# ZechengLi19/CIM

Measured on AMD Instinct MI355X. Metric: images/sec training step (ResNet-50 VOC, ~1k proposals/img) at 1/2/4/8 GPU, higher is better.
Workload: dtype fp32

## Files before the change

cim_amd/csrc/conv1x1.hip:

```cpp
#include "common.h"
#include "../../include/cim_hip.h"

#ifndef CIM_BODY_PRIO_LEVEL
#define CIM_BODY_PRIO_LEVEL 3
#endif
#if CIM_BODY_PRIO_LEVEL > 0
#define CIM_BODY_PRIO() __builtin_amdgcn_s_setprio(CIM_BODY_PRIO_LEVEL)
#else
#define CIM_BODY_PRIO()
#endif
namespace {

#ifndef CIM_SMALL_BK
#define CIM_SMALL_BK 32
#endif
#ifndef CIM_SMALL_ABL
#define CIM_SMALL_ABL 0
#endif
constexpr int SBM = 64, SBN = 64, SBK = CIM_SMALL_BK;
constexpr int SLD = 68;
typedef float f32x16 __attribute__((ext_vector_type(16)));
typedef float f32x4u __attribute__((ext_vector_type(4), aligned(4)));
__device__ __forceinline__ float4 ld4(const float* p) {
    const f32x4u v = *reinterpret_cast<const f32x4u*>(p);
    return make_float4(v.x, v.y, v.z, v.w);
}

struct SmallArgs {
    const float* A; const float* B; float* C; float* Xraw;
    const float* gamma; const float* beta; const float* mean; const float* var; const float* res;
    float eps;
    int M, N, K, lda, ldb, ldc;
    int a_mcontig, b_kcontig, relu, bn;
    int splits; float* ws;
    const float* colbias;
    const float* mask; const float* mgamma; const float* mvar; float meps;
    const float* mxr; const float* mmean; float* mpart; int mparts;
    int res_w, res_ws, res_hw;
};
struct InputBn { const float* y; const float* gamma; const float* var; float eps;
                 const float* xr; const float* mean; float* part; };

typedef unsigned int u32x4 __attribute__((ext_vector_type(4)));
typedef __amdgpu_buffer_rsrc_t rsrc_t;
__device__ __forceinline__ rsrc_t make_rsrc(const float* p, long long floats) {
    return __builtin_amdgcn_make_buffer_rsrc(const_cast<float*>(p), 0, (int)(unsigned)(floats * 4), 0x00020000);
}
__device__ __forceinline__ float4 bld4(rsrc_t r, unsigned byte_off) {
    const u32x4 v = __builtin_amdgcn_raw_buffer_load_b128(r, byte_off, 0, 0);
    return make_float4(__uint_as_float(v.x), __uint_as_float(v.y), __uint_as_float(v.z), __uint_as_float(v.w));
}
__device__ __forceinline__ float bld1(rsrc_t r, unsigned byte_off) {
    return __uint_as_float(__builtin_amdgcn_raw_buffer_load_b32(r, byte_off, 0, 0));
}
constexpr unsigned OOB = 0x7fffffffu;
__host__ __device__ __forceinline__ long long tile_extent(bool RC, int rows, int K, int ld) {
    return RC ? (long long)(K - 1) * ld + rows : (long long)(rows - 1) * ld + K;
}
template <bool RC, int ROWS>
__device__ __forceinline__ unsigned tile_off(int ld, int r0, int k0, int p) {
    int r, k;
    if (RC) { k = k0 + p / (ROWS / 4); r = r0 + (p % (ROWS / 4)) * 4; return ((unsigned)k * ld + r) * 4u; }
    r = r0 + p % ROWS; k = k0 + (p / ROWS) * 4;
    return ((unsigned)r * ld + k) * 4u;
}
template <bool RC, int ROWS>
__device__ __forceinline__ float4 tile_ktail(float4 v, int K, int k0, int p) {
    if (!RC) {
        const int left = K - (k0 + (p / ROWS) * 4);
        v.x = left > 0 ? v.x : 0.0f; v.y = left > 1 ? v.y : 0.0f; v.z = left > 2 ? v.z : 0.0f; v.w = left > 3 ? v.w : 0.0f;
    }
    return v;
}

template <bool RC, int ROWS>
__device__ __forceinline__ void tile_store(float* __restrict__ S, float4 v, int p) {
    if (RC) {
        const int k = p / (ROWS / 4), r = (p % (ROWS / 4)) * 4;
        *reinterpret_cast<float4*>(S + k * SLD + r) = v;
    } else {
        const int r = p % ROWS, k = (p / ROWS) * 4;
        S[(k + 0) * SLD + r] = v.x;
        S[(k + 1) * SLD + r] = v.y;
        S[(k + 2) * SLD + r] = v.z;
        S[(k + 3) * SLD + r] = v.w;
    }
}

__device__ __forceinline__ float small_value(const SmallArgs& g, int row, int col, float v, float& s1, float& s2) {
    const size_t o = (size_t)row * g.ldc + col;
    float y = v;
    if (g.bn) {
        const float a = g.gamma[row] * rsqrtf(g.var[row] + g.eps);
        y = fmaf(v, a, g.beta[row] - g.mean[row] * a);
    }
    if (g.res) {
        if (g.res_w == 0) y += g.res[o];
        else {
            const int py = col / g.res_w, px = col - py * g.res_w;
            if (!((py | px) & 1)) y += g.res[(size_t)row * g.res_hw + (py >> 1) * g.res_ws + (px >> 1)];
        }
    }
    if (g.colbias) y += g.colbias[col];
    if (g.relu) y = fmaxf(y, 0.0f);
    if (g.mask) {
        const bool on = g.mask[o] > 0.0f;
        if (g.mpart && on) { s1 += y; s2 = fmaf(y, g.mxr[o] - g.mmean[row], s2); }
        y = on ? y * (g.mgamma[row] * rsqrtf(g.mvar[row] + g.meps)) : 0.0f;
    }
    return y;
}
__device__ __forceinline__ void small_finish(const SmallArgs& g, int row, int col, float v, float& s1, float& s2) {
    const size_t o = (size_t)row * g.ldc + col;
    if (g.Xraw) g.Xraw[o] = v;
    g.C[o] = small_value(g, row, col, v, s1, s2);
}
__device__ __forceinline__ void small_finish(const SmallArgs& g, int row, int col, float v) {
    float s1 = 0.0f, s2 = 0.0f;
    small_finish(g, row, col, v, s1, s2);
}
__device__ __forceinline__ void small_put_part(const SmallArgs& g, int row, int group, int lane, float s1, float s2) {
#pragma unroll
    for (int o = 16; o > 0; o >>= 1) {
        s1 += __shfl_xor(s1, o);
        s2 += __shfl_xor(s2, o);
    }
    if ((lane & 31) == 0 && row < g.M && group < g.mparts) {
        g.mpart[(size_t)group * g.M + row] = s1;
        g.mpart[((size_t)g.mparts + group) * g.M + row] = s2;
    }
}
__device__ __forceinline__ void small_epilogue(const SmallArgs& g, const f32x16& acc, int row0, int col0, int lane, int split) {
    const int col = col0 + (lane & 31);
    if (g.splits > 1) {
        if (col < g.N) {
#pragma unroll
            for (int r = 0; r < 16; ++r) {
                const int row = row0 + 8 * (r >> 2) + 4 * (lane >> 5) + (r & 3);
                if (row < g.M) g.ws[((size_t)split * g.M + row) * g.N + col] = acc[r];
            }
        }
        return;
    }
    if (g.mpart == nullptr) {
        if (col < g.N) {
#pragma unroll
            for (int r = 0; r < 16; ++r) {
                const int row = row0 + 8 * (r >> 2) + 4 * (lane >> 5) + (r & 3);
                if (row < g.M) small_finish(g, row, col, acc[r]);
            }
        }
        return;
    }
#pragma unroll
    for (int r = 0; r < 16; ++r) {
        const int row = row0 + 8 * (r >> 2) + 4 * (lane >> 5) + (r & 3);
        float s1 = 0.0f, s2 = 0.0f;
        if (col < g.N && row < g.M) small_finish(g, row, col, acc[r], s1, s2);
        small_put_part(g, row, col0 >> 5, lane, s1, s2);
    }
}


template <bool AM, bool BKc, int WN>
__global__ __launch_bounds__(128 * WN) void gemm_small_kernel(const SmallArgs g) {
    CIM_BODY_PRIO();
    constexpr int NT = 128 * WN, BNT = 32 * WN;
    constexpr int PA = SBM * 8 / NT, PB = BNT * 8 / NT;
    __shared__ __attribute__((aligned(16))) float As[2][SBK * SLD];
    __shared__ __attribute__((aligned(16))) float Bs[2][SBK * SLD];
    const int tid = threadIdx.x, lane = tid & 63, wave = tid >> 6;
    const int wm = wave / WN, wn = wave % WN;
    const int tiles_n = (g.N + BNT - 1) / BNT;
    const int tile = blockIdx.x;
    const int m0 = (tile / tiles_n) * SBM, n0 = (tile % tiles_n) * BNT;
    const int split = blockIdx.y;
    const int kper = ((g.K + g.splits - 1) / g.splits + SBK - 1) / SBK * SBK;
    const int kbeg = split * kper, kend = min(g.K, kbeg + kper);
#if CIM_SMALL_ABL == 4
    if (g.M > 0) return;
#endif

    f32x16 acc;
#pragma unroll
    for (int i = 0; i < 16; ++i) acc[i] = 0.0f;

    const rsrc_t RA_ = make_rsrc(g.A, tile_extent(AM, g.M, g.K, g.lda)), RB_ = make_rsrc(g.B, tile_extent(!BKc, g.N, g.K, g.ldb));
    unsigned oa[PA], ob[PB];
#pragma unroll
    for (int i = 0; i < PA; ++i) oa[i] = tile_off<AM, SBM>(g.lda, m0, kbeg, tid + i * NT);
#pragma unroll
    for (int i = 0; i < PB; ++i) ob[i] = tile_off<!BKc, BNT>(g.ldb, n0, kbeg, tid + i * NT);
    const unsigned sa = (AM ? (unsigned)g.lda * SBK : (unsigned)SBK) * 4u, sb = (!BKc ? (unsigned)g.ldb * SBK : (unsigned)SBK) * 4u;
    float4 ra0[PA], rb0[PB], ra1[PA], rb1[PB];
#if CIM_SMALL_ABL == 3
#define SM_GLOAD(RA, RB, S)                                                                                        \
    {                                                                                                              \
        _Pragma("unroll") for (int i = 0; i < PA; ++i) asm volatile("" : "+v"(RA[i].x), "+v"(RA[i].y), "+v"(RA[i].z), "+v"(RA[i].w)); \
        _Pragma("unroll") for (int i = 0; i < PB; ++i) asm volatile("" : "+v"(RB[i].x), "+v"(RB[i].y), "+v"(RB[i].z), "+v"(RB[i].w)); \
    }
#else
#define SM_GLOAD(RA, RB, S)                                                                                        \
    {                                                                                                              \
        _Pragma("unroll") for (int i = 0; i < PA; ++i) RA[i] = bld4(RA_, oa[i] + (unsigned)(S) * sa);               \
        _Pragma("unroll") for (int i = 0; i < PB; ++i) RB[i] = bld4(RB_, ob[i] + (unsigned)(S) * sb);               \
    }
#endif
#define SM_PUT(RA, RB, BUF, S)                                                                                     \
    {                                                                                                              \
        _Pragma("unroll") for (int i = 0; i < PA; ++i)                                                             \
            tile_store<AM, SBM>(As[BUF], tile_ktail<AM, SBM>(RA[i], g.K, kbeg + (S) * SBK, tid + i * NT), tid + i * NT);     \
        _Pragma("unroll") for (int i = 0; i < PB; ++i)                                                             \
            tile_store<!BKc, BNT>(Bs[BUF], tile_ktail<!BKc, BNT>(RB[i], g.K, kbeg + (S) * SBK, tid + i * NT), tid + i * NT); \
    }
#define SM_MMA(BUF)                                                                                                \
    {                                                                                                              \
        const float* __restrict__ a = As[BUF] + (lane >> 5) * SLD + wm * 32 + (lane & 31);                         \
        const float* __restrict__ b = Bs[BUF] + (lane >> 5) * SLD + wn * 32 + (lane & 31);                         \
        float av[SBK / 2], bv[SBK / 2];                                                                            \
        _Pragma("unroll") for (int t = 0; t < SBK / 2; ++t) { av[t] = a[2 * t * SLD]; bv[t] = b[2 * t * SLD]; }    \
        _Pragma("unroll") for (int t = 0; t < (CIM_SMALL_ABL == 1 ? 1 : SBK / 2); ++t)                             \
            acc = __builtin_amdgcn_mfma_f32_32x32x2f32(av[t], bv[t], acc, 0, 0, 0);                                \
        asm volatile("" : "+a"(acc));       \
    }
    if (kbeg < kend) {
        const int nslab = (kend - kbeg + SBK - 1) / SBK;
        const int last = nslab - 1;
        SM_GLOAD(ra0, rb0, 0)
        SM_GLOAD(ra1, rb1, min(1, last))
        SM_PUT(ra0, rb0, 0, 0)
        asm volatile("" : "+a"(acc));
        __syncthreads();
        for (int s = 0; s < nslab; s += 2) {
            SM_GLOAD(ra0, rb0, min(s + 2, last))
            SM_MMA(0)
            if (s + 1 < nslab) SM_PUT(ra1, rb1, 1, s + 1)
            __syncthreads();
            if (s + 1 >= nslab) break;
            SM_GLOAD(ra1, rb1, min(s + 3, last))
            SM_MMA(1)
            if (s + 2 < nslab) SM_PUT(ra0, rb0, 0, s + 2)
            __syncthreads();
        }
    }
#undef SM_GLOAD
#undef SM_PUT
#undef SM_MMA

#if CIM_SMALL_ABL == 2
    if (m0 + wm * 32 + lane < 0) small_epilogue(g, acc, m0 + wm * 32, n0 + wn * 32, lane, split);
#else
    small_epilogue(g, acc, m0 + wm * 32, n0 + wn * 32, lane, split);
#endif
}

__device__ __forceinline__ float splitk_sum(const float* __restrict__ ws, size_t i, size_t mn, int splits) {
    float v = ws[i];
    for (int k0 = 1; k0 < splits; k0 += 8) {
        float p[8];
#pragma unroll
        for (int j = 0; j < 8; ++j) p[j] = k0 + j < splits ? ws[(size_t)(k0 + j) * mn + i] : 0.0f;
#pragma unroll
        for (int j = 0; j < 8; ++j)
            if (k0 + j < splits) v += p[j];
    }
    return v;
}
__global__ __launch_bounds__(256) void small_splitk_reduce_kernel(const SmallArgs g) {
    CIM_BODY_PRIO();
    const size_t i = (size_t)blockIdx.x * 256 + threadIdx.x;
    const size_t mn = (size_t)g.M * g.N;
    if (i >= mn) return;
    small_finish(g, (int)(i / g.N), (int)(i % g.N), splitk_sum(g.ws, i, mn, g.splits));
}
__global__ __launch_bounds__(256) void small_splitk_reduce4_kernel(const SmallArgs g) {
    CIM_BODY_PRIO();
    const size_t q = (size_t)blockIdx.x * 256 + threadIdx.x;
    const size_t mn = (size_t)g.M * g.N;
    const size_t i = q * 4;
    if (i >= mn) return;
    float4 v = *reinterpret_cast<const float4*>(g.ws + i);
    for (int k0 = 1; k0 < g.splits; k0 += 4) {
        float4 p[4];
#pragma unroll
        for (int j = 0; j < 4; ++j)
            p[j] = k0 + j < g.splits ? *reinterpret_cast<const float4*>(g.ws + (size_t)(k0 + j) * mn + i) : make_float4(0.f, 0.f, 0.f, 0.f);
#pragma unroll
        for (int j = 0; j < 4; ++j)
            if (k0 + j < g.splits) { v.x += p[j].x; v.y += p[j].y; v.z += p[j].z; v.w += p[j].w; }
    }
    int row = (int)(i / g.N), col = (int)(i - (size_t)row * g.N);
    const float s[4] = {v.x, v.y, v.z, v.w};
    float y[4], s1 = 0.0f, s2 = 0.0f;
#pragma unroll
    for (int j = 0; j < 4; ++j) {
        y[j] = small_value(g, row, col, s[j], s1, s2);
        if (++col == g.N) { col = 0; ++row; }
    }
    if (g.Xraw) *reinterpret_cast<float4*>(g.Xraw + i) = v;
    *reinterpret_cast<float4*>(g.C + i) = make_float4(y[0], y[1], y[2], y[3]);
}

__global__ __launch_bounds__(256) void small_splitk_reduce_rows_kernel(const SmallArgs g) {
    CIM_BODY_PRIO();
    const int col = blockIdx.x * 256 + threadIdx.x, row = blockIdx.y;
    const size_t mn = (size_t)g.M * g.N;
    float s1 = 0.0f, s2 = 0.0f;
    if (col < g.N) {
        const size_t i = (size_t)row * g.N + col;
        small_finish(g, row, col, splitk_sum(g.ws, i, mn, g.splits), s1, s2);
    }
    small_put_part(g, row, col >> 5, threadIdx.x & 63, s1, s2);
}

struct BnPartTable { cim_bn_part_desc d[24]; int first[25]; int n; };
__global__ __launch_bounds__(256) void bn_part_finish_kernel(const BnPartTable t) {
    CIM_BODY_PRIO();
    __shared__ float sh[2][8][32];
    int e = 0;
    while (e + 1 < t.n && (int)blockIdx.x >= t.first[e + 1]) ++e;
    const cim_bn_part_desc& d = t.d[e];
    const int C = d.channels, parts = d.parts, total = d.images * d.parts;
    const int c = ((int)blockIdx.x - t.first[e]) * 32 + (threadIdx.x & 31), grp = threadIdx.x >> 5;
    float t1 = 0.0f, t2 = 0.0f;
    if (c < C) {
        for (int i0 = grp; i0 < total; i0 += 32) {
            float a[4], b[4];
#pragma unroll
            for (int j = 0; j < 4; ++j) {
                const int i = i0 + 8 * j;
                const int img = i / parts, p = i - img * parts;
                const float* q = d.part + ((size_t)img * 2 * parts + p) * C + c;
                a[j] = i < total ? q[0] : 0.0f;
                b[j] = i < total ? q[(size_t)parts * C] : 0.0f;
            }
#pragma unroll
            for (int j = 0; j < 4; ++j) { t1 += a[j]; t2 += b[j]; }
        }
    }
    sh[0][grp][threadIdx.x & 31] = t1;
    sh[1][grp][threadIdx.x & 31] = t2;
    __syncthreads();
    if (grp == 0 && c < C) {
        float a1 = 0.0f, a2 = 0.0f;
#pragma unroll
        for (int k = 0; k < 8; ++k) { a1 += sh[0][k][threadIdx.x]; a2 += sh[1][k][threadIdx.x]; }
        if (d.dbeta) d.dbeta[c] = a1;
        if (d.dgamma) d.dgamma[c] = a2 * rsqrtf(d.var[c] + d.eps);
    }
}

enum { CONV_FWD = 0, CONV_DX = 1, CONV_DW = 2 };
struct ConvGeom { int H, W, Ho, Wo, stride, cin, cout; float inv_w; int dil; };

#ifndef CIM_CONV3_BK
#define CIM_CONV3_BK 32
#endif
constexpr int CBK = CIM_CONV3_BK;
template <int MODE, int KS = 3>
__global__ __launch_bounds__(256) void conv3x3_small_kernel(const SmallArgs g, const ConvGeom c) {
    CIM_BODY_PRIO();
    constexpr int TAPS = KS * KS;
    constexpr int NT = 256, PA = SBM * (CBK / 4) / NT, PB = SBN * (CBK / 4) / NT;
    extern __shared__ __attribute__((aligned(16))) float c3_smem[];
    float (*As)[CBK * SLD] = reinterpret_cast<float (*)[CBK * SLD]>(c3_smem);
    float (*Bs)[CBK * SLD] = reinterpret_cast<float (*)[CBK * SLD]>(c3_smem + 2 * CBK * SLD);
    const int tid = threadIdx.x, lane = tid & 63, wave = tid >> 6;
    const int wm = wave >> 1, wn = wave & 1;
    const int tiles_n = (g.N + SBN - 1) / SBN;
    const int m0 = (blockIdx.x / tiles_n) * SBM, n0 = (blockIdx.x % tiles_n) * SBN;
    const int split = blockIdx.y;
    const int kper = ((g.K + g.splits - 1) / g.splits + CBK - 1) / CBK * CBK;
    const int kbeg = split * kper, kend = min(g.K, kbeg + kper);

    const rsrc_t RA_ = make_rsrc(g.A, tile_extent(MODE == CONV_DX, g.M, g.K, g.lda));
    const rsrc_t RB_ = make_rsrc(g.B, (long long)(MODE == CONV_DX ? c.cout * c.Ho * c.Wo : c.cin * c.H * c.W));
    const int hw_src = MODE == CONV_DX ? c.Ho * c.Wo : c.H * c.W;
    int py[PB][4], px[PB][4];
    int boff[PB], bdy[PB], bdx[PB];
#pragma unroll
    for (int i = 0; i < PB; ++i) {
        const int p = tid + i * NT;
        if (MODE == CONV_DW) {
            const int n = n0 + p % SBN;
            const int ch = n / TAPS, tap = n - ch * TAPS;
            boff[i] = n < g.N ? ch * hw_src : -1;
            bdy[i] = (tap / KS - KS / 2) * c.dil;
            bdx[i] = (tap - (tap / KS) * KS - KS / 2) * c.dil;
        } else {
            const int wrow = (MODE == CONV_DX) ? c.W : c.Wo;
#pragma unroll
            for (int j = 0; j < 4; ++j) {
                const int n = n0 + (p % 16) * 4 + j;
                const int y = (int)(((float)n + 0.5f) * c.inv_w);
                py[i][j] = n < g.N ? y : -(1 << 20);
                px[i][j] = n - y * wrow;
            }
        }
    }
    unsigned oa[PA];
#pragma unroll
    for (int i = 0; i < PA; ++i) oa[i] = tile_off<MODE == CONV_DX, SBM>(g.lda, m0, kbeg, tid + i * NT);
    const unsigned sa = (MODE == CONV_DX ? (unsigned)g.lda * CBK : (unsigned)CBK) * 4u;

    auto load_b = [&](int k0, float4 (&rb)[PB]) {
#pragma unroll
        for (int i = 0; i < PB; ++i) {
            const int p = tid + i * NT;
            unsigned off[4];
            if (MODE == CONV_DW) {
                const int k = k0 + (p / SBN) * 4;
#pragma unroll
                for (int j = 0; j < 4; ++j) {
                    const int po = k + j;
                    const int yo = (int)(((float)po + 0.5f) * c.inv_w), xo = po - yo * c.Wo;
                    const int yi = yo * c.stride + bdy[i], xi = xo * c.stride + bdx[i];
                    const bool ok = boff[i] >= 0 && po < g.K && (unsigned)yi < (unsigned)c.H && (unsigned)xi < (unsigned)c.W;
                    off[j] = ok ? (unsigned)(boff[i] + yi * c.W + xi) * 4u : OOB;
                }
            } else {
                const int k = k0 + p / 16;
                const int ch = k / TAPS, tap = k - ch * TAPS;
                const int dy = (tap / KS - KS / 2) * c.dil, dx = (tap - (tap / KS) * KS - KS / 2) * c.dil;
                const int base = ch * hw_src;
#pragma unroll
                for (int j = 0; j < 4; ++j) {
                    if (MODE == CONV_DX) {
                        const int ty = py[i][j] - dy, tx = px[i][j] - dx;
                        const int yo = c.stride == 2 ? ty >> 1 : ty, xo = c.stride == 2 ? tx >> 1 : tx;
                        const bool ok = ty >= 0 && tx >= 0 && yo < c.Ho && xo < c.Wo && !(c.stride == 2 && ((ty | tx) & 1));
                        off[j] = ok ? (unsigned)(base + yo * c.Wo + xo) * 4u : OOB;
                    } else {
                        const int yi = py[i][j] * c.stride + dy, xi = px[i][j] * c.stride + dx;
                        const bool ok = (unsigned)yi < (unsigned)c.H && (unsigned)xi < (unsigned)c.W;
                        off[j] = ok ? (unsigned)(base + yi * c.W + xi) * 4u : OOB;
                    }
                }
            }
#if CIM_SMALL_ABL == 3
            asm volatile("" : "+v"(rb[i].x), "+v"(rb[i].y), "+v"(rb[i].z), "+v"(rb[i].w) : "v"(off[0]), "v"(off[1]), "v"(off[2]), "v"(off[3]));
#elif CIM_SMALL_ABL == 5
            rb[i] = make_float4(bld1(RB_, (unsigned)(p * 16 + k0 * 64)), bld1(RB_, (unsigned)(p * 16 + k0 * 64 + 4)),
                                bld1(RB_, (unsigned)(p * 16 + k0 * 64 + 8)), bld1(RB_, (unsigned)(p * 16 + k0 * 64 + 12)));
#else
            rb[i] = make_float4(bld1(RB_, off[0]), bld1(RB_, off[1]), bld1(RB_, off[2]), bld1(RB_, off[3]));
#endif
        }
    };
    auto load_a = [&](int s, float4 (&ra)[PA]) {
#pragma unroll
        for (int i = 0; i < PA; ++i)
            ra[i] = bld4(RA_, oa[i] + (unsigned)s * sa);
    };

    f32x16 acc;
#pragma unroll
    for (int i = 0; i < 16; ++i) acc[i] = 0.0f;
    float4 ra0[PA], rb0[PB], ra1[PA], rb1[PB];
#define C3_PUT(RA, RB, BUF, S)                                                                                      \
    {                                                                                                               \
        _Pragma("unroll") for (int i = 0; i < PA; ++i)                                                              \
            tile_store<MODE == CONV_DX, SBM>(As[BUF], tile_ktail<MODE == CONV_DX, SBM>(RA[i], g.K, kbeg + (S) * CBK, tid + i * NT), tid + i * NT); \
        _Pragma("unroll") for (int i = 0; i < PB; ++i) tile_store<MODE != CONV_DW, SBN>(Bs[BUF], RB[i], tid + i * NT); \
    }
#define C3_MMA(BUF)                                                                                                 \
    {                                                                                                               \
        const float* __restrict__ a = As[BUF] + (lane >> 5) * SLD + wm * 32 + (lane & 31);                          \
        const float* __restrict__ b = Bs[BUF] + (lane >> 5) * SLD + wn * 32 + (lane & 31);                          \
        float av[CBK / 2], bv[CBK / 2];                                                                             \
        _Pragma("unroll") for (int t = 0; t < CBK / 2; ++t) { av[t] = a[2 * t * SLD]; bv[t] = b[2 * t * SLD]; }     \
        _Pragma("unroll") for (int t = 0; t < (CIM_SMALL_ABL == 1 ? 1 : CBK / 2); ++t)                              \
            acc = __builtin_amdgcn_mfma_f32_32x32x2f32(av[t], bv[t], acc, 0, 0, 0);                                 \
        asm volatile("" : "+a"(acc));                                                                               \
    }
    if (kbeg < kend) {
        const int nslab = (kend - kbeg + CBK - 1) / CBK;
        const int last = nslab - 1;
        load_a(0, ra0); load_b(kbeg, rb0);
        load_a(min(1, last), ra1); load_b(kbeg + min(1, last) * CBK, rb1);
        C3_PUT(ra0, rb0, 0, 0)
        asm volatile("" : "+a"(acc));
        __syncthreads();
        for (int s = 0; s < nslab; s += 2) {
            load_a(min(s + 2, last), ra0); load_b(kbeg + min(s + 2, last) * CBK, rb0);
            C3_MMA(0)
            if (s + 1 < nslab) C3_PUT(ra1, rb1, 1, s + 1)
            __syncthreads();
            if (s + 1 >= nslab) break;
            load_a(min(s + 3, last), ra1); load_b(kbeg + min(s + 3, last) * CBK, rb1);
            C3_MMA(1)
            if (s + 2 < nslab) C3_PUT(ra0, rb0, 0, s + 2)
            __syncthreads();
        }
    }
#undef C3_PUT
#undef C3_MMA
#if CIM_SMALL_ABL == 2
    if (m0 + wm * 32 + lane < 0)
#endif
    small_epilogue(g, acc, m0 + wm * 32, n0 + wn * 32, lane, split);
}

struct Dx2Geom { int H, W, Ho, Wo, cin, cout; int first[5]; int tiles_n[4]; int group0[4]; };
struct ColMap { int Wc, W, py, px, Nc, group0; };

__device__ __forceinline__ void small_epilogue_mapped(const SmallArgs& g, const f32x16& acc, int row0, int col0, int lane, const ColMap& cm) {
    const int nc = col0 + (lane & 31);
    const bool in = nc < cm.Nc;
    const int yc = nc / cm.Wc, xc = nc - yc * cm.Wc;
    const int col = (2 * yc + cm.py) * cm.W + 2 * xc + cm.px;
    if (g.mpart == nullptr) {
        if (in) {
#pragma unroll
            for (int r = 0; r < 16; ++r) {
                const int row = row0 + 8 * (r >> 2) + 4 * (lane >> 5) + (r & 3);
                if (row < g.M) small_finish(g, row, col, acc[r]);
            }
        }
        return;
    }
#pragma unroll
    for (int r = 0; r < 16; ++r) {
        const int row = row0 + 8 * (r >> 2) + 4 * (lane >> 5) + (r & 3);
        float s1 = 0.0f, s2 = 0.0f;
        if (in && row < g.M) small_finish(g, row, col, acc[r], s1, s2);
        small_put_part(g, row, cm.group0 + (col0 >> 5), lane, s1, s2);
    }
}

__global__ __launch_bounds__(256) void conv3x3_dx2_kernel(const SmallArgs g, const Dx2Geom c) {
    CIM_BODY_PRIO();
    constexpr int NT = 256, PA = SBM * (CBK / 4) / NT, PB = SBN * (CBK / 4) / NT;
    extern __shared__ __attribute__((aligned(16))) float d2_smem[];
    float (*As)[CBK * SLD] = reinterpret_cast<float (*)[CBK * SLD]>(d2_smem);
    float (*Bs)[CBK * SLD] = reinterpret_cast<float (*)[CBK * SLD]>(d2_smem + 2 * CBK * SLD);
    const int tid = threadIdx.x, lane = tid & 63, wave = tid >> 6;
    const int wm = wave >> 1, wn = wave & 1;
    int cls = 0;
    while (cls < 3 && (int)blockIdx.x >= c.first[cls + 1]) ++cls;
    const int py = cls >> 1, px = cls & 1;
    const int Wc = (c.W - px + 1) >> 1, Nc = ((c.H - py + 1) >> 1) * Wc;
    const int local = (int)blockIdx.x - c.first[cls], tn = c.tiles_n[cls];
    const int m0 = (local / tn) * SBM, n0 = (local % tn) * SBN;
    const int nx = px ? 2 : 1, lgT = py + px, T = 1 << lgT;
    const int K = c.cout << lgT;
    const int nslab = (K + CBK - 1) / CBK;
    const int how = c.Ho * c.Wo;
    const rsrc_t RA_ = make_rsrc(g.A, tile_extent(true, g.M, 9 * c.cout, g.lda));
    const rsrc_t RB_ = make_rsrc(g.B, (long long)c.cout * how);
    int yc[PB][4], xc[PB][4];
#pragma unroll
    for (int i = 0; i < PB; ++i) {
        const int p = tid + i * NT;
#pragma unroll
        for (int j = 0; j < 4; ++j) {
            const int nc = n0 + (p % 16) * 4 + j;
            const int y = nc / Wc;
            yc[i][j] = nc < Nc ? y : -(1 << 20);
            xc[i][j] = nc - y * Wc;
        }
    }
    auto tap_of = [&](int j, int& tap, int& oy, int& ox) {
        const int jy = j / nx, jx = j - jy * nx;
        const int ky = py ? 2 * jy : 1, kx = px ? 2 * jx : 1;
        tap = ky * 3 + kx;
        oy = (py && jy == 0) ? 1 : 0;
        ox = (px && jx == 0) ? 1 : 0;
    };
    auto load_a = [&](int k0, float4 (&ra)[PA]) {
#pragma unroll
        for (int i = 0; i < PA; ++i) {
            const int p = tid + i * NT;
            const int k = k0 + p / (SBM / 4), r = m0 + (p % (SBM / 4)) * 4;
            const int co = k >> lgT;
            int tap, oy, ox;
            tap_of(k & (T - 1), tap, oy, ox);
            ra[i] = bld4(RA_, co < c.cout ? ((unsigned)(co * 9 + tap) * g.lda + r) * 4u : OOB);
        }
    };
    auto load_b = [&](int k0, float4 (&rb)[PB]) {
#pragma unroll
        for (int i = 0; i < PB; ++i) {
            const int p = tid + i * NT;
            const int k = k0 + p / 16;
            const int co = k >> lgT;
            int tap, oy, ox;
            tap_of(k & (T - 1), tap, oy, ox);
            const int base = co * how;
            unsigned off[4];
#pragma unroll
            for (int j = 0; j < 4; ++j) {
                const int yo = yc[i][j] + oy, xo = xc[i][j] + ox;
                const bool ok = co < c.cout && yo >= 0 && yo < c.Ho && xo < c.Wo;
                off[j] = ok ? (unsigned)(base + yo * c.Wo + xo) * 4u : OOB;
            }
            rb[i] = make_float4(bld1(RB_, off[0]), bld1(RB_, off[1]), bld1(RB_, off[2]), bld1(RB_, off[3]));
        }
    };
    f32x16 acc;
#pragma unroll
    for (int i = 0; i < 16; ++i) acc[i] = 0.0f;
    float4 ra0[PA], rb0[PB], ra1[PA], rb1[PB];
#define D2_PUT(RA, RB, BUF)                                                                                         \
    {                                                                                                               \
        _Pragma("unroll") for (int i = 0; i < PA; ++i) tile_store<true, SBM>(As[BUF], RA[i], tid + i * NT);          \
        _Pragma("unroll") for (int i = 0; i < PB; ++i) tile_store<true, SBN>(Bs[BUF], RB[i], tid + i * NT);          \
    }
#define D2_MMA(BUF)                                                                                                 \
    {                                                                                                               \
        const float* __restrict__ a = As[BUF] + (lane >> 5) * SLD + wm * 32 + (lane & 31);                          \
        const float* __restrict__ b = Bs[BUF] + (lane >> 5) * SLD + wn * 32 + (lane & 31);                          \
        float av[CBK / 2], bv[CBK / 2];                                                                             \
        _Pragma("unroll") for (int t = 0; t < CBK / 2; ++t) { av[t] = a[2 * t * SLD]; bv[t] = b[2 * t * SLD]; }     \
        _Pragma("unroll") for (int t = 0; t < CBK / 2; ++t)                                                         \
            acc = __builtin_amdgcn_mfma_f32_32x32x2f32(av[t], bv[t], acc, 0, 0, 0);                                 \
        asm volatile("" : "+a"(acc));                                                                               \
    }
    {
        const int last = nslab - 1;
        load_a(0, ra0); load_b(0, rb0);
        load_a(min(1, last) * CBK, ra1); load_b(min(1, last) * CBK, rb1);
        D2_PUT(ra0, rb0, 0)
        asm volatile("" : "+a"(acc));
        __syncthreads();
        for (int s = 0; s < nslab; s += 2) {
            load_a(min(s + 2, last) * CBK, ra0); load_b(min(s + 2, last) * CBK, rb0);
            D2_MMA(0)
            if (s + 1 < nslab) D2_PUT(ra1, rb1, 1)
            __syncthreads();
            if (s + 1 >= nslab) break;
            load_a(min(s + 3, last) * CBK, ra1); load_b(min(s + 3, last) * CBK, rb1);
            D2_MMA(1)
            if (s + 2 < nslab) D2_PUT(ra0, rb0, 0)
            __syncthreads();
        }
    }
#undef D2_PUT
#undef D2_MMA
    const ColMap cm{Wc, c.W, py, px, Nc, c.group0[cls]};
    small_epilogue_mapped(g, acc, m0 + wm * 32, n0 + wn * 32, lane, cm);
}

__global__ __launch_bounds__(256) void conv3x3_wt_kernel(const float* __restrict__ w, float* __restrict__ wt, int cin) {
    extern __shared__ float wt_s[];
    const int co = blockIdx.x, n = cin * 9;
    for (int i = threadIdx.x; i < n; i += 256) wt_s[i] = w[(size_t)co * n + i];
    __syncthreads();
    for (int i = threadIdx.x; i < n; i += 256) {
        const int tap = i / cin, ci = i - tap * cin;
        wt[(size_t)co * n + i] = wt_s[ci * 9 + tap];
    }
}

struct WtTable { cim_wt_desc d[16]; int first[17]; int n; };
__global__ __launch_bounds__(256) void conv3x3_wt_multi_kernel(const WtTable t) {
    extern __shared__ float wt_s[];
    int e = 0;
    while (e + 1 < t.n && (int)blockIdx.x >= t.first[e + 1]) ++e;
    const int co = blockIdx.x - t.first[e], cin = t.d[e].cin, n = cin * 9;
    const float* __restrict__ w = t.d[e].w;
    float* __restrict__ wt = t.d[e].wt;
    for (int i = threadIdx.x; i < n; i += 256) wt_s[i] = w[(size_t)co * n + i];
    __syncthreads();
    for (int i = threadIdx.x; i < n; i += 256) {
        const int tap = i / cin, ci = i - tap * cin;
        wt[(size_t)co * n + i] = wt_s[ci * 9 + tap];
    }
}

static void set_input_bn(SmallArgs& g, const InputBn* in_bn) {
    if (in_bn == nullptr) return;
    g.mask = in_bn->y; g.mgamma = in_bn->gamma; g.mvar = in_bn->var; g.meps = in_bn->eps;
    g.mxr = in_bn->xr; g.mmean = in_bn->mean; g.mpart = in_bn->part; g.mparts = (g.N + 31) / 32;
}
static void launch_splitk_reduce(const SmallArgs& g, hipStream_t st) {
    if (g.mpart) {
        hipLaunchKernelGGL(small_splitk_reduce_rows_kernel, dim3((unsigned)((g.N + 255) / 256), (unsigned)g.M), dim3(256), 0, st, g);
    } else {
        const size_t n = (size_t)g.M * g.N;
        if (n >= (1u << 19) && g.ldc == g.N && n % 4 == 0 && (((size_t)g.ws | (size_t)g.C | (size_t)g.Xraw) & 15) == 0)
            hipLaunchKernelGGL(small_splitk_reduce4_kernel, dim3((unsigned)((n / 4 + 255) / 256)), dim3(256), 0, st, g);
        else
            hipLaunchKernelGGL(small_splitk_reduce_kernel, dim3((unsigned)((n + 255) / 256)), dim3(256), 0, st, g);
    }
}

template <bool AM, bool BKc>
static void launch_small(const SmallArgs& g, int splits, hipStream_t st, bool narrow) {
    const long long tm = (g.M + SBM - 1) / SBM;
    if (narrow)
        hipLaunchKernelGGL((gemm_small_kernel<AM, BKc, 1>), dim3((unsigned)(tm * ((g.N + 31) / 32)), (unsigned)splits), dim3(128), 0, st, g);
    else
        hipLaunchKernelGGL((gemm_small_kernel<AM, BKc, 2>), dim3((unsigned)(tm * ((g.N + 63) / 64)), (unsigned)splits), dim3(256), 0, st, g);
}

}

extern "C" int cim_gemm_small_splits(int M, int N, int K) {
    const long long tiles = (long long)((M + SBM - 1) / SBM) * ((N + SBN - 1) / SBN);
#ifndef CIM_SMALL_WGS
#define CIM_SMALL_WGS 512
#endif
#ifndef CIM_SMALL_MINSLABS
#define CIM_SMALL_MINSLABS 4
#endif
    constexpr int min_k = CIM_SMALL_MINSLABS * SBK, want = CIM_SMALL_WGS;
    int s = 1;
    while (tiles * s < want && K / (s * 2) >= min_k && s < 64) s *= 2;
    return s;
}

static int gemm_small_impl(const float* A, const float* B, float* C, int M, int N, int K, int lda, int ldb, int ldc,
                           int a_mcontig, int b_kcontig, float* x_raw, const float* gamma, const float* beta,
                           const float* mean, const float* var, float eps, const float* residual, int relu, int splits,
                           float* workspace, void* stream, const InputBn* in_bn, int res_w = 0);

extern "C" int cim_gemm_small_f32(const float* A, const float* B, float* C, int M, int N, int K, int lda, int ldb, int ldc,
                                  int a_mcontig, int b_kcontig, float* x_raw, const float* gamma, const float* beta,
                                  const float* mean, const float* var, float eps, const float* residual, int relu, int splits,
                                  float* workspace, void* stream) {
    return gemm_small_impl(A, B, C, M, N, K, lda, ldb, ldc, a_mcontig, b_kcontig, x_raw, gamma, beta, mean, var, eps, residual, relu,
                           splits, workspace, stream, nullptr);
}

static int gemm_small_impl(const float* A, const float* B, float* C, int M, int N, int K, int lda, int ldb, int ldc,
                           int a_mcontig, int b_kcontig, float* x_raw, const float* gamma, const float* beta,
                           const float* mean, const float* var, float eps, const float* residual, int relu, int splits,
                           float* workspace, void* stream, const InputBn* in_bn, int res_w) {
    CIM_CHECK_ARG(res_w == 0 || (residual && res_w > 0 && N % res_w == 0 && ldc == N));
    CIM_CHECK_ARG(A && B && C && M > 0 && N > 0 && K > 0 && lda > 0 && ldb > 0 && ldc >= N && splits >= 1);
    CIM_CHECK_ARG((gamma == nullptr) == (beta == nullptr) && (gamma == nullptr) == (mean == nullptr) && (gamma == nullptr) == (var == nullptr));
    CIM_CHECK_ARG(splits == 1 || workspace);
    SmallArgs g{};
    g.A = A; g.B = B; g.C = C; g.Xraw = x_raw;
    g.gamma = gamma; g.beta = beta; g.mean = mean; g.var = var; g.res = residual; g.eps = eps;
    g.M = M; g.N = N; g.K = K; g.lda = lda; g.ldb = ldb; g.ldc = ldc;
    g.a_mcontig = a_mcontig; g.b_kcontig = b_kcontig; g.relu = relu; g.bn = gamma != nullptr;
    g.splits = splits; g.ws = workspace; g.colbias = nullptr;
    g.res_w = res_w;
    if (res_w) { g.res_ws = (res_w + 1) / 2; g.res_hw = ((N / res_w + 1) / 2) * g.res_ws; }
    set_input_bn(g, in_bn);
    const long long tiles = (long long)((M + SBM - 1) / SBM) * ((N + SBN - 1) / SBN);
    CIM_CHECK_ARG(tiles * 2 < (1ll << 31) && splits <= 65535 && M <= 65535);
    CIM_CHECK_ARG(tile_extent(a_mcontig != 0, M, K, lda) < (1ll << 29) && tile_extent(b_kcontig == 0, N, K, ldb) < (1ll << 29));
    const bool narrow = tiles * splits < 128;
    hipStream_t st = cim::as_stream(stream);
    if (a_mcontig) {
        if (b_kcontig) launch_small<true, true>(g, splits, st, narrow); else launch_small<true, false>(g, splits, st, narrow);
    } else {
        if (b_kcontig) launch_small<false, true>(g, splits, st, narrow); else launch_small<false, false>(g, splits, st, narrow);
    }
    if (splits > 1) launch_splitk_reduce(g, st);
    CIM_CHECK_LAUNCH();
    return 0;
}

extern "C" int cim_linear_bias_f32(const float* X, const float* W, const float* bias, float* Y, int M, int N, int K, int splits,
                                   float* workspace, void* stream) {
    CIM_CHECK_ARG(X && W && Y && M > 0 && N > 0 && K > 0 && splits >= 1 && splits <= 65535 && (splits == 1 || workspace));
    SmallArgs g{};
    g.A = X; g.B = W; g.C = Y; g.Xraw = nullptr;
    g.gamma = g.beta = g.mean = g.var = g.res = nullptr; g.eps = 0.f;
    g.M = M; g.N = N; g.K = K; g.lda = K; g.ldb = K; g.ldc = N;
    g.a_mcontig = 0; g.b_kcontig = 1; g.relu = 0; g.bn = 0;
    g.splits = splits; g.ws = workspace; g.colbias = bias;
    hipStream_t st = cim::as_stream(stream);
    launch_small<false, true>(g, splits, st, false);
    if (splits > 1) {
        const size_t n = (size_t)M * N;
        hipLaunchKernelGGL(small_splitk_reduce_kernel, dim3((unsigned)((n + 255) / 256)), dim3(256), 0, st, g);
    }
    CIM_CHECK_LAUNCH();
    return 0;
}

extern "C" long long cim_conv1x1_bwd_workspace(int B, int cin, int cout, int hw) {
    const long long dx = (long long)cim_gemm_small_splits(cin, hw, cout) * cin * hw;
    const long long dw = (long long)cim_gemm_small_splits(cout, cin, hw) * cout * cin + (B > 1 ? (long long)cout * cin : 0);
    const long long dconv = (long long)B * cout * hw;
    return (long long)sizeof(float) * (dconv + dx + dw);
}

namespace {
struct ForkJoin {
    hipStream_t main, side;
    hipEvent_t ev_fork, ev_join;
    bool on;
    ForkJoin(hipStream_t m, hipStream_t s, void* fork_event, void* join_event, bool want)
        : main(m), side(s), ev_fork(static_cast<hipEvent_t>(fork_event)), ev_join(static_cast<hipEvent_t>(join_event)),
          on(want && s != nullptr && s != m) {}
    hipStream_t fork() {
        if (!on) return main;
        (void)hipEventRecord(ev_fork, main);
        (void)hipStreamWaitEvent(side, ev_fork, 0);
        return side;
    }
    void join() {
        if (!on) return;
        (void)hipEventRecord(ev_join, side);
        (void)hipStreamWaitEvent(main, ev_join, 0);
    }
};

__global__ __launch_bounds__(256) void small_axpy_kernel(float* __restrict__ y, const float* __restrict__ x, size_t n) {
    const size_t i = (size_t)blockIdx.x * 256 + threadIdx.x;
    if (i < n) y[i] += x[i];
}
}

extern "C" int cim_conv1x1_bn_act_bwd(const float* dy, const float* y, const float* x_raw, const float* x, const float* w,
                                      const float* gamma, const float* mean, const float* var, float eps, int relu,
                                      float* dres, float* dgamma, float* dbeta, float* dx, float* dw, int B, int cin, int cout,
                                      int hw, float* workspace, void* stream, void* side_stream, void* fork_event, void* join_event, int join,
                                      int dy_is_dconv, const float* in_gamma, const float* in_var, float in_eps,
                                      const float* in_xr, const float* in_mean, float* in_part, const float* dx_add, int dx_add_w) {
    CIM_CHECK_ARG(dx_add_w == 0 || (dx_add != nullptr && dx_add_w > 0 && hw % dx_add_w == 0));
    CIM_CHECK_ARG(side_stream == nullptr || side_stream == stream || (fork_event != nullptr && (!join || join_event != nullptr)));
    const size_t add_bs = dx_add_w ? (size_t)cin * ((hw / dx_add_w + 1) / 2) * ((dx_add_w + 1) / 2) : (size_t)cin * hw;
    CIM_CHECK_ARG(dy && x_raw && x && w && gamma && mean && var && workspace && B > 0 && cin > 0 && cout > 0 && hw > 0);
    CIM_CHECK_ARG(dx_add == nullptr || (dx != nullptr && in_gamma == nullptr));
    CIM_CHECK_ARG((y != nullptr || !relu) && ((dgamma == nullptr) == (dbeta == nullptr)));
    CIM_CHECK_ARG(!dy_is_dconv || (dres == nullptr && dgamma == nullptr));
    CIM_CHECK_ARG((in_gamma == nullptr) == (in_var == nullptr));
    CIM_CHECK_ARG(in_part == nullptr || (in_gamma && in_xr && in_mean));
    float* dconv = dy_is_dconv ? const_cast<float*>(dy) : workspace;
    float* ws_dx = workspace + (size_t)B * cout * hw;
    float* ws_dw = ws_dx + (size_t)cim_gemm_small_splits(cin, hw, cout) * cin * hw;
    int rc = dy_is_dconv ? 0 : cim_bn_act_bwd(dy, y, x_raw, gamma, mean, var, eps, dconv, dres, dgamma, dbeta, B, cout, hw, relu, stream);
    if (rc) return rc;
    ForkJoin fj(cim::as_stream(stream), cim::as_stream(side_stream), fork_event, join_event, dx && dw);
    void* st_dw = fj.fork();
    for (int b = 0; b < B && dw; ++b) {
        const int sp = cim_gemm_small_splits(cout, cin, hw);
        float* out = b == 0 ? dw : ws_dw + (size_t)sp * cout * cin;
        rc = cim_gemm_small_f32(dconv + (size_t)b * cout * hw, x + (size_t)b * cin * hw, out, cout, cin, hw, hw, hw, cin, 0, 1,
// ... 138 lines not shown
        t.first[t.n] = total;
        hipLaunchKernelGGL(bn_part_finish_kernel, dim3((unsigned)total), dim3(256), 0, st, t);
    }
    CIM_CHECK_LAUNCH();
    return 0;
}

extern "C" int cim_conv3x3_wt_multi(const cim_wt_desc* descs, int n, void* stream) {
    CIM_CHECK_ARG(descs && n > 0);
    hipStream_t st = cim::as_stream(stream);
    for (int base = 0; base < n; base += 16) {
        WtTable t{};
        t.n = n - base < 16 ? n - base : 16;
        int total = 0, max_cin = 0;
        for (int i = 0; i < t.n; ++i) {
            const cim_wt_desc& d = descs[base + i];
            CIM_CHECK_ARG(d.w && d.wt && d.cin > 0 && d.cout > 0 && (size_t)d.cin * 9 * sizeof(float) <= 64 * 1024);
            t.d[i] = d;
            t.first[i] = total;
            total += d.cout;
            max_cin = d.cin > max_cin ? d.cin : max_cin;
        }
        t.first[t.n] = total;
        const size_t lds = sizeof(float) * max_cin * 9;
        if (lds > 48 * 1024) {
            hipError_t e = hipFuncSetAttribute(reinterpret_cast<const void*>(conv3x3_wt_multi_kernel), hipFuncAttributeMaxDynamicSharedMemorySize, (int)lds);
            if (e != hipSuccess) return (int)e;
        }
        hipLaunchKernelGGL(conv3x3_wt_multi_kernel, dim3((unsigned)total), dim3(256), lds, st, t);
    }
    CIM_CHECK_LAUNCH();
    return 0;
}

extern "C" int cim_conv3x3_nchw_bn_act_bwd(const float* dy, const float* y, const float* x_raw, const float* x, const float* w,
                                      const float* gamma, const float* mean, const float* var, float eps, int relu,
                                      float* dres, float* dgamma, float* dbeta, float* dx, float* dw, int B, int cin, int cout,
                                      int H, int W, int stride, int dilation, float* workspace, void* stream, void* side_stream,
                                      void* fork_event, void* join_event, int join, int dy_is_dconv, const float* in_gamma, const float* in_var, float in_eps,
                                      const float* in_xr, const float* in_mean, float* in_part, const float* wt_ready) {
    CIM_CHECK_ARG(dy && x_raw && x && w && gamma && mean && var && workspace && B > 0);
    CIM_CHECK_ARG(side_stream == nullptr || side_stream == stream || (fork_event != nullptr && (!join || join_event != nullptr)));
    CONV3_ARGS_OK(4);
    CIM_CHECK_ARG((y != nullptr || !relu) && ((dgamma == nullptr) == (dbeta == nullptr)) && cout % 4 == 0);
    CIM_CHECK_ARG(!dy_is_dconv || (dres == nullptr && dgamma == nullptr));
    CIM_CHECK_ARG((in_gamma == nullptr) == (in_var == nullptr));
    CIM_CHECK_ARG(in_part == nullptr || (in_gamma && in_xr && in_mean));
    const ConvGeom cx = conv_geom(cin, cout, H, W, stride, CONV_DX, dilation), cw = conv_geom(cin, cout, H, W, stride, CONV_DW, dilation);
    const int hwo = cx.Ho * cx.Wo, hw = H * W;
    hipStream_t st = cim::as_stream(stream);
    float* dconv = dy_is_dconv ? const_cast<float*>(dy) : workspace;
    float* wt_own = workspace + (size_t)B * cout * hwo;
    const float* wt = wt_ready ? wt_ready : wt_own;
    float* ws_dx = wt_own + (size_t)cout * cin * 9;
    float* ws_dw = ws_dx + (size_t)cim_gemm_small_splits(cin, hw, 9 * cout) * cin * hw;
    CIM_CHECK_ARG((size_t)cin * 9 * sizeof(float) <= 64 * 1024);
    int rc = dy_is_dconv ? 0 : cim_bn_act_bwd(dy, y, x_raw, gamma, mean, var, eps, dconv, dres, dgamma, dbeta, B, cout, hwo, relu, stream);
    if (rc) return rc;
    ForkJoin fj(st, cim::as_stream(side_stream), fork_event, join_event, dx && dw);
    hipStream_t st_dw = fj.fork();
    for (int b = 0; b < B && dw; ++b) {
        const int sp = cim_gemm_small_splits(cout, 9 * cin, hwo);
        float* out = b == 0 ? dw : ws_dw + (size_t)sp * cout * cin * 9;
        conv3x3_launch(CONV_DW, dconv + (size_t)b * cout * hwo, x + (size_t)b * cin * hw, out, cout, 9 * cin, hwo, hwo, 9 * cin, cw,
                       nullptr, nullptr, nullptr, nullptr, nullptr, 0.f, nullptr, 0, sp, ws_dw, st_dw);
        if (b) {
            const size_t n = (size_t)cout * cin * 9;
            hipLaunchKernelGGL(small_axpy_kernel, dim3((unsigned)((n + 255) / 256)), dim3(256), 0, st_dw, dw, out, n);
        }
    }
    if (dx && !wt_ready) hipLaunchKernelGGL(conv3x3_wt_kernel, dim3(cout), dim3(256), sizeof(float) * cin * 9, st, w, wt_own, cin);
    const int parts = cim_conv3x3_dx_parts(H, W, dilation == 1 ? stride : 1);
    for (int b = 0; b < B && dx; ++b) {
        const InputBn ib{x + (size_t)b * cin * hw, in_gamma, in_var, in_eps, in_xr ? in_xr + (size_t)b * cin * hw : nullptr, in_mean,
                         in_part ? in_part + (size_t)b * 2 * parts * cin : nullptr};
        if (stride == 2 && dilation == 1) {
            SmallArgs g{};
            g.A = wt; g.B = dconv + (size_t)b * cout * hwo; g.C = dx + (size_t)b * cin * hw;
            g.M = cin; g.N = hw; g.K = 9 * cout; g.lda = cin; g.ldb = 0; g.ldc = hw;
            g.splits = 1;
            set_input_bn(g, in_gamma ? &ib : nullptr);
            g.mparts = parts;
            const Dx2Geom c2 = dx2_geom(cin, cout, H, W);
            const size_t lds = sizeof(float) * 4 * CBK * SLD;
            if (lds > 48 * 1024) {
                hipError_t e = hipFuncSetAttribute(reinterpret_cast<const void*>(conv3x3_dx2_kernel), hipFuncAttributeMaxDynamicSharedMemorySize, (int)lds);
                if (e != hipSuccess) return (int)e;
            }
            hipLaunchKernelGGL(conv3x3_dx2_kernel, dim3((unsigned)c2.first[4]), dim3(256), lds, st, g, c2);
            continue;
        }
        conv3x3_launch(CONV_DX, wt, dconv + (size_t)b * cout * hwo, dx + (size_t)b * cin * hw, cin, hw, 9 * cout, cin, hw, cx, nullptr,
                       nullptr, nullptr, nullptr, nullptr, 0.f, nullptr, 0, cim_gemm_small_splits(cin, hw, 9 * cout), ws_dx, st, 3,
                       in_gamma ? &ib : nullptr);
    }
    if (join) fj.join();
    CIM_CHECK_LAUNCH();
    return 0;
}
```

Baseline: 79.36.

## Deepen small GEMM/conv3x3 register pipeline with BK16 and fold split-K in-kernel

Changes the small-tile GEMM and 3x3 conv kernels from a two-deep register prefetch with 32-wide K slabs to a configurable four-deep prefetch with 16-wide slabs. The aim is to hide more global-load latency while keeping register pressure bounded. It also adds a 'fold' mode: for large tile counts, one block walks every split-K range itself and sums in registers, removing the workspace writes and the separate reduce kernel. The cost is less parallelism in that case and more barriers per unit of K. The dx2 kernel keeps its own 32-wide K slab.

```diff
diff --git a/cim_amd/csrc/conv1x1.hip b/cim_amd/csrc/conv1x1.hip
--- a/cim_amd/csrc/conv1x1.hip
+++ b/cim_amd/csrc/conv1x1.hip
@@ -12,12 +12,17 @@
 namespace {
 
 #ifndef CIM_SMALL_BK
-#define CIM_SMALL_BK 32
+#define CIM_SMALL_BK 16
+#endif
+#ifndef CIM_SMALL_DEPTH
+#define CIM_SMALL_DEPTH 4
 #endif
 #ifndef CIM_SMALL_ABL
 #define CIM_SMALL_ABL 0
 #endif
-constexpr int SBM = 64, SBN = 64, SBK = CIM_SMALL_BK;
+constexpr int SBM = 64, SBN = 64, SBK = CIM_SMALL_BK, SDEPTH = CIM_SMALL_DEPTH;
+constexpr int SKQ = 32;
+static_assert((SBK == 16 || SBK == 32) && SKQ % SBK == 0 && SDEPTH >= 2, "small-tile pipeline switches");
 constexpr int SLD = 68;
 typedef float f32x16 __attribute__((ext_vector_type(16)));
 typedef float f32x4u __attribute__((ext_vector_type(4), aligned(4)));
@@ -33,6 +38,7 @@
     int M, N, K, lda, ldb, ldc;
     int a_mcontig, b_kcontig, relu, bn;
     int splits; float* ws;
+    int fold;
     const float* colbias;
     const float* mask; const float* mgamma; const float* mvar; float meps;
     const float* mxr; const float* mmean; float* mpart; int mparts;
@@ -132,7 +138,7 @@
 }
 __device__ __forceinline__ void small_epilogue(const SmallArgs& g, const f32x16& acc, int row0, int col0, int lane, int split) {
     const int col = col0 + (lane & 31);
-    if (g.splits > 1) {
+    if (g.splits > 1 && !g.fold) {
         if (col < g.N) {
 #pragma unroll
             for (int r = 0; r < 16; ++r) {
@@ -166,7 +172,8 @@
 __global__ __launch_bounds__(128 * WN) void gemm_small_kernel(const SmallArgs g) {
     CIM_BODY_PRIO();
     constexpr int NT = 128 * WN, BNT = 32 * WN;
-    constexpr int PA = SBM * 8 / NT, PB = BNT * 8 / NT;
+    constexpr int PA = SBM * (SBK / 4) / NT, PB = BNT * (SBK / 4) / NT;
+    static_assert(PA >= 1 && PB >= 1 && PA * NT == SBM * (SBK / 4) && PB * NT == BNT * (SBK / 4), "tile pieces");
     __shared__ __attribute__((aligned(16))) float As[2][SBK * SLD];
     __shared__ __attribute__((aligned(16))) float Bs[2][SBK * SLD];
     const int tid = threadIdx.x, lane = tid & 63, wave = tid >> 6;
@@ -175,13 +182,15 @@
     const int tile = blockIdx.x;
     const int m0 = (tile / tiles_n) * SBM, n0 = (tile % tiles_n) * BNT;
     const int split = blockIdx.y;
-    const int kper = ((g.K + g.splits - 1) / g.splits + SBK - 1) / SBK * SBK;
-    const int kbeg = split * kper, kend = min(g.K, kbeg + kper);
+    const int kper = ((g.K + g.splits - 1) / g.splits + SKQ - 1) / SKQ * SKQ;
 #if CIM_SMALL_ABL == 4
     if (g.M > 0) return;
 #endif
 
-    f32x16 acc;
+    f32x16 acc, sum;
+    const int range_end = g.fold ? g.splits : split + 1;
+    for (int range = split; range < range_end; ++range) {
+    const int kbeg = range * kper, kend = min(g.K, kbeg + kper);
 #pragma unroll
     for (int i = 0; i < 16; ++i) acc[i] = 0.0f;
 
@@ -192,7 +201,7 @@
 #pragma unroll
     for (int i = 0; i < PB; ++i) ob[i] = tile_off<!BKc, BNT>(g.ldb, n0, kbeg, tid + i * NT);
     const unsigned sa = (AM ? (unsigned)g.lda * SBK : (unsigned)SBK) * 4u, sb = (!BKc ? (unsigned)g.ldb * SBK : (unsigned)SBK) * 4u;
-    float4 ra0[PA], rb0[PB], ra1[PA], rb1[PB];
+    float4 ra[SDEPTH][PA], rb[SDEPTH][PB];
 #if CIM_SMALL_ABL == 3
 #define SM_GLOAD(RA, RB, S)                                                                                        \
     {                                                                                                              \
@@ -226,31 +235,37 @@
     if (kbeg < kend) {
         const int nslab = (kend - kbeg + SBK - 1) / SBK;
         const int last = nslab - 1;
-        SM_GLOAD(ra0, rb0, 0)
-        SM_GLOAD(ra1, rb1, min(1, last))
-        SM_PUT(ra0, rb0, 0, 0)
+#pragma unroll
+        for (int d = 0; d < SDEPTH; ++d) SM_GLOAD(ra[d], rb[d], min(d, last))
+        SM_PUT(ra[0], rb[0], 0, 0)
         asm volatile("" : "+a"(acc));
         __syncthreads();
-        for (int s = 0; s < nslab; s += 2) {
-            SM_GLOAD(ra0, rb0, min(s + 2, last))
-            SM_MMA(0)
-            if (s + 1 < nslab) SM_PUT(ra1, rb1, 1, s + 1)
-            __syncthreads();
-            if (s + 1 >= nslab) break;
-            SM_GLOAD(ra1, rb1, min(s + 3, last))
-            SM_MMA(1)
-            if (s + 2 < nslab) SM_PUT(ra0, rb0, 0, s + 2)
-            __syncthreads();
+        for (int s0 = 0; s0 < nslab; s0 += SDEPTH) {
+#pragma unroll
+            for (int u = 0; u < SDEPTH; ++u) {
+                const int s = s0 + u;
+                SM_GLOAD(ra[u], rb[u], min(s + SDEPTH, last))
+                SM_MMA(s & 1)
+                if (s + 1 < nslab) SM_PUT(ra[(u + 1) % SDEPTH], rb[(u + 1) % SDEPTH], (s + 1) & 1, s + 1)
+                __syncthreads();
+                if (s + 1 >= nslab) break;
+            }
         }
     }
 #undef SM_GLOAD
 #undef SM_PUT
 #undef SM_MMA
+    if (range == split) sum = acc;
+    else {
+#pragma unroll
+        for (int i = 0; i < 16; ++i) sum[i] += acc[i];
+    }
+    }
 
 #if CIM_SMALL_ABL == 2
-    if (m0 + wm * 32 + lane < 0) small_epilogue(g, acc, m0 + wm * 32, n0 + wn * 32, lane, split);
+    if (m0 + wm * 32 + lane < 0) small_epilogue(g, sum, m0 + wm * 32, n0 + wn * 32, lane, split);
 #else
-    small_epilogue(g, acc, m0 + wm * 32, n0 + wn * 32, lane, split);
+    small_epilogue(g, sum, m0 + wm * 32, n0 + wn * 32, lane, split);
 #endif
 }
 
@@ -354,9 +369,13 @@
 struct ConvGeom { int H, W, Ho, Wo, stride, cin, cout; float inv_w; int dil; };
 
 #ifndef CIM_CONV3_BK
-#define CIM_CONV3_BK 32
-#endif
-constexpr int CBK = CIM_CONV3_BK;
+#define CIM_CONV3_BK 16
+#endif
+#ifndef CIM_CONV3_DEPTH
+#define CIM_CONV3_DEPTH 4
+#endif
+constexpr int CBK = CIM_CONV3_BK, CDEPTH = CIM_CONV3_DEPTH;
+static_assert((CBK == 16 || CBK == 32) && SKQ % CBK == 0 && CDEPTH >= 2, "3 x 3 pipeline switches");
 template <int MODE, int KS = 3>
 __global__ __launch_bounds__(256) void conv3x3_small_kernel(const SmallArgs g, const ConvGeom c) {
     CIM_BODY_PRIO();
@@ -370,7 +389,7 @@
     const int tiles_n = (g.N + SBN - 1) / SBN;
     const int m0 = (blockIdx.x / tiles_n) * SBM, n0 = (blockIdx.x % tiles_n) * SBN;
     const int split = blockIdx.y;
-    const int kper = ((g.K + g.splits - 1) / g.splits + CBK - 1) / CBK * CBK;
+    const int kper = ((g.K + g.splits - 1) / g.splits + SKQ - 1) / SKQ * SKQ;
     const int kbeg = split * kper, kend = min(g.K, kbeg + kper);
 
     const rsrc_t RA_ = make_rsrc(g.A, tile_extent(MODE == CONV_DX, g.M, g.K, g.lda));
@@ -456,7 +475,7 @@
     f32x16 acc;
 #pragma unroll
     for (int i = 0; i < 16; ++i) acc[i] = 0.0f;
-    float4 ra0[PA], rb0[PB], ra1[PA], rb1[PB];
+    float4 ra[CDEPTH][PA], rb[CDEPTH][PB];
 #define C3_PUT(RA, RB, BUF, S)                                                                                      \
     {                                                                                                               \
         _Pragma("unroll") for (int i = 0; i < PA; ++i)                                                              \
@@ -476,21 +495,21 @@
     if (kbeg < kend) {
         const int nslab = (kend - kbeg + CBK - 1) / CBK;
         const int last = nslab - 1;
-        load_a(0, ra0); load_b(kbeg, rb0);
-        load_a(min(1, last), ra1); load_b(kbeg + min(1, last) * CBK, rb1);
-        C3_PUT(ra0, rb0, 0, 0)
+#pragma unroll
+        for (int d = 0; d < CDEPTH; ++d) { load_a(min(d, last), ra[d]); load_b(kbeg + min(d, last) * CBK, rb[d]); }
+        C3_PUT(ra[0], rb[0], 0, 0)
         asm volatile("" : "+a"(acc));
         __syncthreads();
-        for (int s = 0; s < nslab; s += 2) {
-            load_a(min(s + 2, last), ra0); load_b(kbeg + min(s + 2, last) * CBK, rb0);
-            C3_MMA(0)
-            if (s + 1 < nslab) C3_PUT(ra1, rb1, 1, s + 1)
-            __syncthreads();
-            if (s + 1 >= nslab) break;
-            load_a(min(s + 3, last), ra1); load_b(kbeg + min(s + 3, last) * CBK, rb1);
-            C3_MMA(1)
-            if (s + 2 < nslab) C3_PUT(ra0, rb0, 0, s + 2)
-            __syncthreads();
+        for (int s0 = 0; s0 < nslab; s0 += CDEPTH) {
+#pragma unroll
+            for (int u = 0; u < CDEPTH; ++u) {
+                const int s = s0 + u;
+                load_a(min(s + CDEPTH, last), ra[u]); load_b(kbeg + min(s + CDEPTH, last) * CBK, rb[u]);
+                C3_MMA(s & 1)
+                if (s + 1 < nslab) C3_PUT(ra[(u + 1) % CDEPTH], rb[(u + 1) % CDEPTH], (s + 1) & 1, s + 1)
+                __syncthreads();
+                if (s + 1 >= nslab) break;
+            }
         }
     }
 #undef C3_PUT
@@ -501,6 +520,7 @@
     small_epilogue(g, acc, m0 + wm * 32, n0 + wn * 32, lane, split);
 }
 
+constexpr int D2BK = 32;
 struct Dx2Geom { int H, W, Ho, Wo, cin, cout; int first[5]; int tiles_n[4]; int group0[4]; };
 struct ColMap { int Wc, W, py, px, Nc, group0; };
 
@@ -530,10 +550,10 @@
 
 __global__ __launch_bounds__(256) void conv3x3_dx2_kernel(const SmallArgs g, const Dx2Geom c) {
     CIM_BODY_PRIO();
-    constexpr int NT = 256, PA = SBM * (CBK / 4) / NT, PB = SBN * (CBK / 4) / NT;
+    constexpr int NT = 256, PA = SBM * (D2BK / 4) / NT, PB = SBN * (D2BK / 4) / NT;
     extern __shared__ __attribute__((aligned(16))) float d2_smem[];
-    float (*As)[CBK * SLD] = reinterpret_cast<float (*)[CBK * SLD]>(d2_smem);
-    float (*Bs)[CBK * SLD] = reinterpret_cast<float (*)[CBK * SLD]>(d2_smem + 2 * CBK * SLD);
+    float (*As)[D2BK * SLD] = reinterpret_cast<float (*)[D2BK * SLD]>(d2_smem);
+    float (*Bs)[D2BK * SLD] = reinterpret_cast<float (*)[D2BK * SLD]>(d2_smem + 2 * D2BK * SLD);
     const int tid = threadIdx.x, lane = tid & 63, wave = tid >> 6;
     const int wm = wave >> 1, wn = wave & 1;
     int cls = 0;
@@ -544,7 +564,7 @@
     const int m0 = (local / tn) * SBM, n0 = (local % tn) * SBN;
     const int nx = px ? 2 : 1, lgT = py + px, T = 1 << lgT;
     const int K = c.cout << lgT;
-    const int nslab = (K + CBK - 1) / CBK;
+    const int nslab = (K + D2BK - 1) / D2BK;
     const int how = c.Ho * c.Wo;
     const rsrc_t RA_ = make_rsrc(g.A, tile_extent(true, g.M, 9 * c.cout, g.lda));
     const rsrc_t RB_ = make_rsrc(g.B, (long long)c.cout * how);
@@ -610,26 +630,26 @@
     {                                                                                                               \
         const float* __restrict__ a = As[BUF] + (lane >> 5) * SLD + wm * 32 + (lane & 31);                          \
         const float* __restrict__ b = Bs[BUF] + (lane >> 5) * SLD + wn * 32 + (lane & 31);                          \
-        float av[CBK / 2], bv[CBK / 2];                                                                             \
-        _Pragma("unroll") for (int t = 0; t < CBK / 2; ++t) { av[t] = a[2 * t * SLD]; bv[t] = b[2 * t * SLD]; }     \
-        _Pragma("unroll") for (int t = 0; t < CBK / 2; ++t)                                                         \
+        float av[D2BK / 2], bv[D2BK / 2];                                                                             \
+        _Pragma("unroll") for (int t = 0; t < D2BK / 2; ++t) { av[t] = a[2 * t * SLD]; bv[t] = b[2 * t * SLD]; }     \
+        _Pragma("unroll") for (int t = 0; t < D2BK / 2; ++t)                                                         \
             acc = __builtin_amdgcn_mfma_f32_32x32x2f32(av[t], bv[t], acc, 0, 0, 0);                                 \
         asm volatile("" : "+a"(acc));                                                                               \
     }
     {
         const int last = nslab - 1;
         load_a(0, ra0); load_b(0, rb0);
-        load_a(min(1, last) * CBK, ra1); load_b(min(1, last) * CBK, rb1);
+        load_a(min(1, last) * D2BK, ra1); load_b(min(1, last) * D2BK, rb1);
         D2_PUT(ra0, rb0, 0)
         asm volatile("" : "+a"(acc));
         __syncthreads();
         for (int s = 0; s < nslab; s += 2) {
-            load_a(min(s + 2, last) * CBK, ra0); load_b(min(s + 2, last) * CBK, rb0);
+            load_a(min(s + 2, last) * D2BK, ra0); load_b(min(s + 2, last) * D2BK, rb0);
             D2_MMA(0)
             if (s + 1 < nslab) D2_PUT(ra1, rb1, 1)
             __syncthreads();
             if (s + 1 >= nslab) break;
-            load_a(min(s + 3, last) * CBK, ra1); load_b(min(s + 3, last) * CBK, rb1);
+            load_a(min(s + 3, last) * D2BK, ra1); load_b(min(s + 3, last) * D2BK, rb1);
             D2_MMA(1)
             if (s + 2 < nslab) D2_PUT(ra0, rb0, 0)
             __syncthreads();
@@ -704,7 +724,7 @@
 #ifndef CIM_SMALL_MINSLABS
 #define CIM_SMALL_MINSLABS 4
 #endif
-    constexpr int min_k = CIM_SMALL_MINSLABS * SBK, want = CIM_SMALL_WGS;
+    constexpr int min_k = CIM_SMALL_MINSLABS * SKQ, want = CIM_SMALL_WGS;
     int s = 1;
     while (tiles * s < want && K / (s * 2) >= min_k && s < 64) s *= 2;
     return s;
@@ -743,14 +763,22 @@
     const long long tiles = (long long)((M + SBM - 1) / SBM) * ((N + SBN - 1) / SBN);
     CIM_CHECK_ARG(tiles * 2 < (1ll << 31) && splits <= 65535 && M <= 65535);
     CIM_CHECK_ARG(tile_extent(a_mcontig != 0, M, K, lda) < (1ll << 29) && tile_extent(b_kcontig == 0, N, K, ldb) < (1ll << 29));
-    const bool narrow = tiles * splits < 128;
+#ifndef CIM_SMALL_FOLD_TILES
+#define CIM_SMALL_FOLD_TILES 256
+#endif
+#ifndef CIM_SMALL_FOLD_XRAW
+#define CIM_SMALL_FOLD_XRAW 0
+#endif
+    g.fold = splits > 1 && tiles >= CIM_SMALL_FOLD_TILES && (CIM_SMALL_FOLD_XRAW || x_raw == nullptr);
+    const int grid_y = g.fold ? 1 : splits;
+    const bool narrow = tiles * grid_y < 128;
     hipStream_t st = cim::as_stream(stream);
     if (a_mcontig) {
-        if (b_kcontig) launch_small<true, true>(g, splits, st, narrow); else launch_small<true, false>(g, splits, st, narrow);
+        if (b_kcontig) launch_small<true, true>(g, grid_y, st, narrow); else launch_small<true, false>(g, grid_y, st, narrow);
     } else {
-        if (b_kcontig) launch_small<false, true>(g, splits, st, narrow); else launch_small<false, false>(g, splits, st, narrow);
-    }
-    if (splits > 1) launch_splitk_reduce(g, st);
+        if (b_kcontig) launch_small<false, true>(g, grid_y, st, narrow); else launch_small<false, false>(g, grid_y, st, narrow);
+    }
+    if (splits > 1 && !g.fold) launch_splitk_reduce(g, st);
     CIM_CHECK_LAUNCH();
     return 0;
 }
@@ -1055,7 +1083,7 @@
             set_input_bn(g, in_gamma ? &ib : nullptr);
             g.mparts = parts;
             const Dx2Geom c2 = dx2_geom(cin, cout, H, W);
-            const size_t lds = sizeof(float) * 4 * CBK * SLD;
+            const size_t lds = sizeof(float) * 4 * D2BK * SLD;
             if (lds > 48 * 1024) {
                 hipError_t e = hipFuncSetAttribute(reinterpret_cast<const void*>(conv3x3_dx2_kernel), hipFuncAttributeMaxDynamicSharedMemorySize, (int)lds);
                 if (e != hipSuccess) return (int)e;
```

Result: no change. 79.26, median of 3 (-0.1%).
